# IntptrMax/YoloSharp

Measured on AMD Instinct MI355X. Metric: train images/sec YOLOv8n 640x640 bs=64/GPU, higher is better.
Workload: dtype bf16; 1 GPU; YOLOv8n detect train step (fwd+loss+bwd+AdamW), 64x3x640x640 per GPU, COCO-80 synthetic labels; global_batch=64, parallelism=dp1

## Files before the change

### yolosharp_amd/csrc/conv.hip

```cpp
#include "ys_internal.h"
#include "ys_kernels.h"
#include <atomic>
#include <cstdlib>
#include <map>
#include <mutex>
#include <vector>

template <class T, int MR, int NR, int NW>
__device__ inline void conv_epilogue(const ConvArgs& a, f32x4 (&acc)[MR][NR], const long (&orow)[MR], const bool (&mv)[MR],
                                     int n0, T* wst, float* sStat, long stat_row) {
  constexpr int EPL = Elem<T>::EPL;
  constexpr int BN = NR * 16;
  constexpr int BNP = BN + EPL;
  constexpr int VPP = BN / EPL;
  constexpr int NIT = (16 * VPP + 63) / 64;
  const int tid = threadIdx.x, lane = tid & 63, wave = tid >> 6, li = lane & 15, q = lane >> 4;
  const bool do_stats = a.stats != nullptr;
  float s1[NR][4], s2[NR][4];
#pragma unroll
  for (int nf = 0; nf < NR; nf++)
#pragma unroll
    for (int r = 0; r < 4; r++) { s1[nf][r] = 0.f; s2[nf][r] = 0.f; }
  char* yb = (char*)a.y;
  const char* rb = (const char*)a.res;
// ... 381 lines not shown
        }
#pragma unroll
        for (int nf = 0; nf < NR; nf++) {
          const uint4 wf = sW[(nf * 16 + li) * wpitch + wbase + (kh * 3 + kw) * 4 + q];
#pragma unroll
          for (int mf = 0; mf < MR; mf++) acc[mf][nf] = ys_mma<T>(wf, xf[mf], acc[mf][nf]);
        }
      }
    }
    if (chunk == nchunks - 1 && !(a.dbg & 4)) {
      __syncthreads();
      long orow[MR];
#pragma unroll
      for (int mf = 0; mf < MR; mf++) orow[mf] = (long)b * a.out_bstride + (pv[mf] ? ((long)poy[mf] * a.Wout + pox[mf]) : 0);
      T* wst = (T*)sP + wave * (16 * (BN + EPL));
      conv_epilogue<T, MR, NR, C3_THREADS / 64>(a, acc, orow, pv, n0, wst, sStat, (long)tile);
    }
    tile = ntile; chunk = nchunk;
  }
}

#include "conv_epi.h"
constexpr int YS_EPI_BATCH_P2 = 4;

#ifdef YS_P2_ABLATE
#define P2_DBG(bit) ((a.dbg & (bit)) != 0)
#else
#define P2_DBG(bit) false
#endif
constexpr int P2_KG = 2;
#define P2_NPU 12
struct P2Tag0 { static constexpr int value = 0; };
struct P2Tag1 { static constexpr int value = 1; };
__host__ __device__ constexpr int p2_reg_group(int mr, int nr, bool tight = false) {
  const int want = mr * nr >= 10 ? 1 : (mr * nr >= 6 ? 2 : 4);
  const int cap = (tight ? 8 : 16) / (mr + nr);
  const int g = want < cap ? want : cap;
  return g >= 4 ? 4 : (g >= 2 ? 2 : 1);
}
struct P2Args {
  int TH, TW, tiles_x, tiles_y, ntiles, PH, PW;
  int ppb;
  int prb;
  int wpitch;
  int nsteps;
  int nsp;
// ... 343 lines not shown
    if (WRES) ys_barrier_lds();
    TL_STAMP();

    const int rh = a.out_rh ? a.out_rh : a.Wout, rw = a.out_rh ? a.out_rw : 1;
    const int tbase = b * (int)a.out_bstride + oy0 * rh + ox0 * rw + (int)a.out_r0;
    int orow[MR];
    bool pv[MR];
#pragma unroll
    for (int mf = 0; mf < MR; mf++) {
      pv[mf] = (bool)((int)(pty[mf] < g.TH) & (int)(oy0 + pty[mf] < a.Hout) & (int)(ox0 + ptx[mf] < a.Wout));
      orow[mf] = tbase + prow[mf];
    }
    char* stg = sPb + wave * (16 * MR * (BN + 8) * 2 + 16 * MR * 16);
    if (F8) {
      const float dq = a.deq[0];
#pragma unroll
      for (int mf = 0; mf < MR; mf++)
#pragma unroll
        for (int nf = 0; nf < NR; nf++)
#pragma unroll
          for (int r = 0; r < 4; r++) acc[mf][nf][r] *= dq;
    }
#ifdef YS_P2_TIMELINE
    if (!P2_DBG(4)) p2_epilogue<MR, NR, RED, YS_EPI_BATCH_P2>(a, acc, orow, pv, n0, stg, st1, st2, [&]() { TL_STAMP(); });
#else
    if (!P2_DBG(4)) p2_epilogue<MR, NR, RED, YS_EPI_BATCH_P2>(a, acc, orow, pv, n0, stg, st1, st2);
#endif
    TL_STAMP();
    txi = ntx; tyi = nty; b = nb;
  }
  YS_WAIT_VM0();
  if (RED ? a.nred > 0 : a.stats != nullptr) p2_stats_flush<NR, NWV>(a, n0, st1, st2, (float*)sPb, (long)vbx);
  if (F8 && a.amax && blockIdx.y == 0) ys_amax_update(a.amax, amx);
  TL_STAMP();
#ifdef YS_P2_TIMELINE
  if (tl_p) tl_p[0] = (unsigned long long)tl_n;
#endif
}

template <int MR, int NR, int WRES, int NPU, int NT, int F8, int RED = 0>
__global__ void __launch_bounds__(NT, (NT == 512 ? 4 : (NPU <= 6 && MR * NR <= 8 && !F8 ? 3 : 2)))
conv_p2_kernel(ConvArgs a, P2Args g, const int* __restrict__ tab) {
  conv_p2_body<MR, NR, WRES, NPU, NT, F8, RED>(a, g, tab, (int)blockIdx.x, (int)gridDim.x);
}

struct P2Prob { ConvArgs a; P2Args g; const int* tab; };
struct P2Group { int n; int end[YS_GROUP_MAX]; P2Prob p[YS_GROUP_MAX]; };
template <int MR, int NR, int WRES, int NPU, int NT, int RED>
__global__ void __launch_bounds__(NT, (NT == 512 ? 4 : (NPU <= 6 && MR * NR <= 8 ? 3 : 2)))
// ... 299 lines not shown
  YS_LAUNCH_LDS((conv_p2_kernel<MR, NR, WRES, NPU, NT, F8, RED>), dim3(p.gx, p.gy), NT, p.lds, st, a, p.g, tab);
#ifdef YS_P2_TIMELINE
  if (tl_path) {
    static unsigned long long h[64 * 64];
    hipStreamSynchronize(st);
    hipMemcpy(h, tl_buf, sizeof(h), hipMemcpyDeviceToHost);
    FILE* f = fopen(tl_path, "a");
    if (f) {
      fprintf(f, "# k%d%d s%d cin%d cout%d M%d mr%d nr%d wres%d npu%d tile%dx%d grid%dx%d lds%d ntiles%d nsteps%d\n", a.KH, a.KW, a.SA, a.Cin, a.Cout, a.M, MR, NR, WRES, NPU, p.g.TH, p.g.TW, p.gx, p.gy, (int)p.lds, p.g.ntiles, p.g.nsteps);
      for (int w = 0; w < 64 && w * 37 < p.gx; w++) {
        const int n = (int)h[w * 64];
        if (n <= 0) continue;
        fprintf(f, "wg%d:", w * 37);
        for (int i = 1; i < n; i++) fprintf(f, " %llu", h[w * 64 + 1 + i] - h[w * 64 + 1]);
        fprintf(f, "\n");
      }
      fclose(f);
    }
  }
#endif
  return YS_OK;
}
static int conv_p2_group_dispatch(hipStream_t st, const ConvArgs* a, const P2Plan* p, int n, const int* gxs, size_t lds);
static int conv_p2_dispatch(hipStream_t st, const ConvArgs& a, const P2Plan& p) {
  {
#define P2F(M_, N_, F_, R_) { \
    if (p.wres) return p.npu == 6 ? conv_p2_launch_t<M_, N_, 1, 6, 256, F_, R_>(st, a, p) : conv_p2_launch_t<M_, N_, 1, 12, 256, F_, R_>(st, a, p); \
    return p.npu == 6 ? conv_p2_launch_t<M_, N_, 0, 6, 256, F_, R_>(st, a, p) : conv_p2_launch_t<M_, N_, 0, 12, 256, F_, R_>(st, a, p); }
#define P2(M_, N_) if (p.mr == M_ && p.nr == N_) { if (a.f8) P2F(M_, N_, 1, 0) else if (a.nred > 0) P2F(M_, N_, 0, 1) else P2F(M_, N_, 0, 0) }
    if (a.f8 && a.nred > 0) { ys_set_error("conv p2: the fused BN-backward reduction has no fp8 variant"); return YS_ERR_UNSUPPORTED; }
#ifdef YS_P2_ONE
#ifndef YS_P2_ONE_M
#define YS_P2_ONE_M 1
#define YS_P2_ONE_N 5
#endif
    P2(YS_P2_ONE_M, YS_P2_ONE_N)
#else
    P2(1, 1) P2(2, 1) P2(4, 1) P2(1, 2) P2(2, 2) P2(4, 2) P2(1, 3) P2(2, 3) P2(4, 3) P2(1, 4) P2(2, 4) P2(4, 4) P2(1, 5) P2(2, 5)
#endif
#undef P2
#undef P2F
  }
  ys_set_error("conv p2: no kernel for NT=%d MR=%d NR=%d", p.nt, p.mr, p.nr);
  return YS_ERR_UNSUPPORTED;
}


template <int MR, int NR, int WRES, int NPU, int NT, int RED>
static int conv_p2_group_launch_t(hipStream_t st, const ConvArgs* a, const P2Plan* p, int n, const int* gxs, size_t lds) {
#ifdef YS_P2_ABLATE
  const int dbg = (int)YS_OPT_INT("DBG", 0);
#else
  const int dbg = 0;
#endif
  static std::atomic<unsigned> attr_done{0};
  int dev_id = 0;
  (void)hipGetDevice(&dev_id);
  if (!(attr_done.load(std::memory_order_relaxed) & (1u << (dev_id & 31)))) {
    hipFuncSetAttribute((const void*)conv_p2_group_kernel<MR, NR, WRES, NPU, NT, RED>, hipFuncAttributeMaxDynamicSharedMemorySize, 160 * 1024);
    attr_done.fetch_or(1u << (dev_id & 31), std::memory_order_relaxed);
  }
  P2Group grp{};
  grp.n = n;
// ... 308 lines not shown
    else { if (rows_only) return 0; const int rc = conv_launch_dtype<bf16_t>(st, q); if (rc != YS_OK) return rc; }
  }
  return rows_only ? row0 - a.red_row0 : YS_OK;
}

int ys_conv_bnred_rows(const ConvArgs& a, int dtype) {
  if (dtype != YS_BF16) return 0;
  if (conv_f8_declined(a)) { ConvArgs b = a; b.f8 = 0; return ys_conv_bnred_rows(b, dtype); }
  const bool phases = ys_conv_dgrad_uses_phases(dtype, a.KH, a.DIVM + 1) && a.KW == a.KH;
  if (a.f8 && !a.x8 && a.q8 && ys_conv_wants_x8(a)) { ConvArgs b = a; b.x8 = a.q8; return ys_conv_bnred_rows(b, dtype); }
  if (phases) return conv_dgrad_s2_phases(nullptr, a, true);
  if (a.f8) {
    if (a.x8 && ys_conv_gemm_rows(a)) return a.f8 == 2 ? ys_conv_gemm_rows(a) : 0;
    const P2Plan pf = conv_p2_plan(a);
    if (pf.ok) return 0;
    ConvArgs b = a; b.f8 = 0;
    return ys_conv_bnred_rows(b, dtype);
  }
  if (ys_conv_gemm_rows(a)) return ys_conv_gemm_rows(a);
  const P2Plan p2 = conv_p2_plan(a);
  return p2.ok ? p2.gx : 0;
}

bool ys_conv_wants_x8(const ConvArgs& a) {
  if (!a.f8 || a.x8 || a.in_bstride != (long)a.Hin * a.Win) return false;
  ConvArgs b = a; b.x8 = a.x;
  if (ys_conv_dgrad_uses_phases(YS_BF16, a.KH, a.DIVM + 1) && a.KW == a.KH) {
    for (int ph = 0; ph < 4; ph++) { ConvArgs q; if (conv_dgrad_s2_phase_args(b, ph, q) && ys_conv_gemm_rows(q) != 0) return true; }
    return false;
  }
  return ys_conv_gemm_rows(b) != 0;
}

int ys_conv_launch(hipStream_t st, int dtype, const ConvArgs& a) {
  const int epl = dtype == YS_BF16 ? 8 : 4;
  if (a.Cin % epl || a.in_ldc % epl || a.in_coff % epl) {
    ys_set_error("conv: Cin/ldc/coff (%d,%d,%d) must be multiples of %d", a.Cin, a.in_ldc, a.in_coff, epl);
    return YS_ERR_INVALID_ARG;
  }
  if (dtype == YS_BF16) {
    if (conv_f8_declined(a)) { ConvArgs b = a; b.f8 = 0; return ys_conv_launch(st, dtype, b); }
    const bool phases = ys_conv_dgrad_uses_phases(dtype, a.KH, a.DIVM + 1) && a.KW == a.KH;
    if (a.f8 && !a.x8 && a.q8) {
      ConvArgs b = a; b.x8 = a.q8;
      if (ys_conv_wants_x8(a)) {
        const int rc = ys_f8_quant_view_launch(st, a.f8 == 2 ? 1 : 0, a.x, (long)a.B * a.Hin * a.Win, a.Cin, a.in_ldc, a.in_coff, a.qscale, a.q8, a.amax);
// ... 37 lines not shown
```

### yolosharp_amd/csrc/conv_epi.h

```cpp
#pragma once
#include "ys_internal.h"
#include "ys_kernels.h"

#ifdef YS_P2_ABLATE
#define EPI_DBG(bit) ((a.dbg & (bit)) != 0)
#else
#define EPI_DBG(bit) false
#endif

#include <type_traits>
template <int I, int N, class F> __device__ inline void ys_static_for(F&& f) {
  if constexpr (I < N) { f(std::integral_constant<int, I>{}); ys_static_for<I + 1, N>(f); }
}

#ifdef YS_EMU_BUILD
typedef const BnRedSeg* ys_redp_t;
__device__ inline ys_redp_t ys_red_table(const ConvArgs& a) { return a.red; }
#else
typedef const BnRedSeg __attribute__((address_space(4)))* ys_redp_t;
__device__ inline ys_redp_t ys_red_table(const ConvArgs& a) {
  const char __attribute__((address_space(4)))* ka = (const char __attribute__((address_space(4)))*)__builtin_amdgcn_kernarg_segment_ptr();
  ys_redp_t p = (ys_redp_t)(ka + a.red_koff);
  asm volatile("" : "+s"(p));
  return p;
}
#endif

__device__ inline void ys_bnred_put(const ConvArgs& a, int c, int which, long row, float t) {
  const ys_redp_t rt = ys_red_table(a);
#pragma unroll
  for (int k = 0; k < YS_BNRED_MAXSEG; k++)
    if (k < a.nred && c >= rt[k].c0 && c < rt[k].c1) {
      const int pc = c - rt[k].c0 + rt[k].yc0;
      rt[k].part[(((long)a.red_row0 + row) * 2 + which) * rt[k].C + pc] = t;
    }
}

__host__ __device__ constexpr int p2_epi_stores(int mr, int nr) { return (16 * mr + 64 / (nr * 2) - 1) / (64 / (nr * 2)); }
template <int M> struct EpiMode { static constexpr int value = M; };
struct YsNoStamp { __device__ inline void operator()() const {} };
template <int MR, int NR, int RED = 0, int BMAX = 4 , class SF = YsNoStamp>
__device__ inline void p2_epilogue(const ConvArgs& a, f32x4 (&acc)[MR][NR], const int (&orow)[MR], const bool (&pv)[MR],
                                   int n0, char* stg, float (&s1)[8], float (&s2)[8], SF stamp = SF()) {
  typedef bf16_t T;
  constexpr int BN = NR * 16;
  constexpr int PITCH = (BN + 8) * 2;
  constexpr int NPX = 16 * MR;
  constexpr int VPP = BN / 8;
  constexpr int PPI = 64 / VPP;
  constexpr int NITER = (NPX + PPI - 1) / PPI;
  static_assert(NITER == p2_epi_stores(MR, NR), "p2_epi_stores");
  const int lane = threadIdx.x & 63, li = lane & 15, q = lane >> 4;
  unsigned* rowtab = (unsigned*)(stg + NPX * PITCH);
  const int cv = lane % VPP, pl = lane / VPP;
  const bool active = lane < PPI * VPP;
  const int c = n0 + cv * 8;
  if (q == 0) {
#pragma unroll
    for (int mf = 0; mf < MR; mf++) {
      rowtab[mf * 16 + li] = pv[mf] ? ((unsigned)orow[mf] * (unsigned)a.out_ldc + (unsigned)a.out_coff) * 2u : YS_BUF_OOB;
      rowtab[NPX + mf * 16 + li] = (unsigned)orow[mf];
    }
  }
  const bool red_on = RED != 0 && a.nred > 0;
  const char* ry = nullptr; const float* rscp = nullptr; const float* rshp = nullptr; int rC = 0, rcol = 0; bool ract = false;
  uint4 yv[RED ? NITER : 1];
  float rsc[8], rsh[8];
  if (RED && red_on) {
#pragma unroll
    for (int k = 0; k < YS_BNRED_MAXSEG; k++)
      if (k < a.nred && active && c >= a.red[k].c0 && c < a.red[k].c1) {
        ry = (const char*)a.red[k].y; rscp = a.red[k].scale; rshp = a.red[k].shift; rC = a.red[k].C;
        rcol = c - a.red[k].c0 + a.red[k].yc0; ract = a.red[k].act != 0;
      }
    ys_wave_sync();
#pragma unroll
    for (int it = 0; it < NITER; it++) {
      const int px = it * PPI + pl;
      yv[it] = ys_zero16();
      if (ry && px < NPX && rowtab[px] != YS_BUF_OOB) yv[it] = ys_ld16(ry + ((long)rowtab[NPX + px] * rC + rcol) * 2L);
    }
#pragma unroll
    for (int e = 0; e < 8; e++) { rsc[e] = 0.f; rsh[e] = 0.f; }
    if (ry) { ys_ldcoef<8>(rscp + rcol, rsc); ys_ldcoef<8>(rshp + rcol, rsh); }
  }
  constexpr bool ACC_PRE = RED != 0 && NITER <= BMAX;
  uint4 ov[ACC_PRE ? NITER : 1];
  if (ACC_PRE && a.accumulate) {
    const ys_rsrcv_t rsO = ys_make_rsrcv(a.y, 0x7ffffff0u);
    if (!red_on) ys_wave_sync();
#pragma unroll
    for (int it = 0; it < NITER; it++) {
      const int px = it * PPI + pl;
      const unsigned ro = (active && px < NPX && c < a.Cout) ? rowtab[px] : YS_BUF_OOB;
      ov[it] = ys_bufld16(rsO, ro != YS_BUF_OOB ? ro + (unsigned)c * 2u : YS_BUF_OOB);
    }
  }
  stamp();
#pragma unroll
  for (int mf = 0; mf < MR; mf++) {
#pragma unroll
    for (int nf = 0; nf < NR; nf++) {
      const int c = n0 + nf * 16 + 4 * q;
      float v[4];
#pragma unroll
      for (int r = 0; r < 4; r++) v[r] = acc[mf][nf][r];
      if (!RED && !a.scale && a.shift) {
#pragma unroll
        for (int r = 0; r < 4; r++) {
          const int cc = (c + r) < a.Cout ? (c + r) : 0;
          v[r] += a.shift[cc];
        }
        if (a.act) {
#pragma unroll
          for (int r = 0; r < 4; r++) v[r] = ys_silu(v[r]);
        }
#pragma unroll
        for (int r = 0; r < 4; r++) if (c + r >= a.Cout) v[r] = 0.f;
// ... 40 lines not shown
        }
        if (bn_eval) {
#pragma unroll
          for (int e = 0; e < 8; e++) f[e] = f[e] * sc[e] + sh[e];
          if (a.act) {
#pragma unroll
            for (int e = 0; e < 8; e++) f[e] = ys_silu(f[e]);
          }
#pragma unroll
          for (int e = 0; e < 8; e++) if (c + e >= a.Cout) f[e] = 0.f;
          if (!(rb || accum)) val = ys_pack<T>(f);
        }
        T* yp = (T*)(yb + rofs + c * 2);
        if (rb || accum) {
          float gq[8];
          if (rb) {
            const long row = (long)rowtab[NPX + px];
            ys_unpack<T>(ys_ld16(rb + (row * a.res_ldc + a.res_coff + c) * 2L), gq);
#pragma unroll
            for (int e = 0; e < 8; e++) f[e] += gq[e];
          }
          if (accum) {
            if constexpr (ACC_PRE) ys_unpack<T>(ov[ACC_PRE ? it : 0], gq); else ys_unpack<T>(ys_ld16(yp), gq);
#pragma unroll
            for (int e = 0; e < 8; e++) f[e] += gq[e];
          }
          val = ys_pack<T>(f);
        }
        if (RED && red_on && ry && !EPI_DBG(512)) {
          float g[8], yf[8];
          ys_unpack<T>(val, g);
          ys_unpack<T>(yv[RED ? it : 0], yf);
          if (ract) {
#pragma unroll
            for (int e = 0; e < 8; e++) g[e] *= ys_silu_grad(yf[e] * rsc[e] + rsh[e]);
          }
#pragma unroll
          for (int e = 0; e < 8; e++) { s1[e] += g[e]; s2[e] += g[e] * yf[e]; }
        }
      }
    }
    ys_bufst16(rsY, (rofs != YS_BUF_OOB && !EPI_DBG(256)) ? rofs + (unsigned)c * 2u : YS_BUF_OOB, val);
  };
  if (EPI_DBG(1024)) { ys_wave_sync(); return; }
#pragma unroll
  for (int it = 0; it < NITER; it++) store_iter(it, EpiMode<2>{});
// ... 300 lines not shown
```

### yolosharp_amd/csrc/core.hip

```cpp
#include "ys_internal.h"
#include "ys_kernels.h"
#include <cstring>

static thread_local char g_err[1024] = "";

#include <mutex>
#include <cstdlib>
extern char** environ;
namespace {
const char* const kOptKeys[] = {"ATTN_MFMA", "BNRED", "BNRED_LOG", "BN_ATOMIC", "F8_MIN_CIN", "F8_MIN_TAPS", "GEMM_HALO", "GEMM_MIN_CIN", "GEMM_MIN_M", "GROUP", "HALO_MAX_GRID",
                                "HALO_MIN_FILL", "HALO_MR4", "HEAD_FUSE", "OVERLAP", "SPPF_FUSE", "STEM_BNB_FUSE", "STEM_DIRECT", "WGEMM_KT", "WGEMM_MIN_M", "DBG", "GEMM_DBG"};
bool opt_known(const std::string& k) {
  for (const char* n : kOptKeys) if (k == n) return true;
  return false;
}
struct OptTable {
  std::mutex mu;
  std::map<std::string, double> v;
  std::atomic<unsigned> version{1};
  OptTable() {
    for (char** e = environ; e && *e; e++) {
      if (strncmp(*e, "YS_", 3) != 0) continue;
      const char* eq = strchr(*e, '=');
      if (!eq || eq == *e + 3) continue;
      const std::string key(*e + 3, (size_t)(eq - (*e + 3)));
      if (!opt_known(key)) continue;
      char* end = nullptr;
      const double d = strtod(eq + 1, &end);
      if (end && end != eq + 1 && *end == 0) v[key] = d;
    }
  }
};
OptTable& opt_table() { static OptTable t; return t; }
}
// ... 365 lines not shown
```

### yolosharp_amd/csrc/model.hip

```cpp
#include "ys_model.h"
#include <cstring>
#include <algorithm>

namespace ysm {

static float* chan_ptr(ys_model* m, const ConvL& c, int which) { return m->chan + c.ch_off + (long)which * ((c.cout + 3) / 4 * 4); }
static char* y_ptr(const ys_model* m, const ConvL& c) { return (char*)m->y_all + (size_t)c.y_off * m->es; }
struct ResView { const void* p = nullptr; int ldc = 0, coff = 0; };
static ResView res_view(const ys_model* m, const ConvL& c) {
  if (!c.has_res) return ResView{};
  return ResView{m->bufs[c.res.buf].act, m->bufs[c.res.buf].ldc, c.res.coff};
}
static BnFinProb bn_fin(ys_model* m, const ConvL& c, const float* partial, int nblk, long count) {
  return BnFinProb{partial, nblk, c.cout, (double)count, m->params + c.g_off, m->params + c.b_off, m->state + c.rm_off, m->state + c.rv_off,
                   m->state + c.nbt_off, chan_ptr(m, c, 0), chan_ptr(m, c, 1), chan_ptr(m, c, 2), chan_ptr(m, c, 3)};
}
static int bn_finalize(ys_model* m, const ConvL& c, const float* partial, int nblk, long count) {
  const BnFinProb p = bn_fin(m, c, partial, nblk, count);
  return ys_bn_finalize_launch(m->ctx->stream, partial, nblk, c.cout, count, p.gamma, p.beta, BN_EPS, BN_MOMENTUM, p.run_mean, p.run_var, p.nbt,
                               p.scale, p.shift, p.mean, p.rstd);
}

static int run_dwconv_fwd(ys_model* m, const ConvL& c, int B) {
  hipStream_t st = m->ctx->stream;
// ... 482 lines not shown
      } else {
        rg = rb.grad; rgl = rb.ldc; rgc = c.res.coff;
      }
    }
    const bool fused = bnred_ready(c);
    if (c.pool_next) {
      const Buf& pb = m->bufs[m->pool_buf];
      const int HW = c.Hout * c.Wout;
      if ((long)B * 2 * c.cout > m->n_stat) { ys_set_error("backward: batch %d too large for the Classify statistics rows", B); return YS_ERR_STATE; }
      YS_TRY(ys_cls_bn_bwd_reduce_launch(st, m->dtype, pb.grad, pb.ldc, y, B, HW, c.cout, chan_ptr(m, c, 0), chan_ptr(m, c, 1), c.act ? 1 : 0,
                                         m->stat_partial));
      YS_TRY(bn_bwd_finalize(m, c, B, M));
      void* dyb = (m->overlap && c.dy_own) ? c.dy_own : m->dy_scratch;
      YS_TRY(ys_cls_bn_bwd_apply_launch(st, m->dtype, pb.grad, pb.ldc, y, B, HW, c.cout, chan_ptr(m, c, 0), chan_ptr(m, c, 1), chan_ptr(m, c, 4),
                                        chan_ptr(m, c, 5), c.act ? 1 : 0, dyb));
      dy = dyb; dy_ldc = c.cout; dy_coff = 0;
    } else {
    c.red_seen = 0;
    void* rg_apply = nullptr;
    if (fused) {
      const ChanFinProb p = bn_bwd_fin(m, c, bnred_src(m, c), M);
      YS_TRY(ys_bn_bwd_finalize_src_launch(st, p.src, c.cout, M, p.g0, p.g1, p.c1, p.c2, p.scale, p.mean, p.rstd));
      rg_apply = rg;
    } else {
      int nblk = 0;
      YS_TRY(ys_bn_bwd_reduce_launch(st, m->dtype, ob.grad, ob.ldc, c.out.coff, y, M, c.cout, chan_ptr(m, c, 0), chan_ptr(m, c, 1),
                                     chan_ptr(m, c, 2), chan_ptr(m, c, 3), c.act ? 1 : 0, rg, rgl, rgc, m->stat_partial, &nblk));
      YS_TRY(bn_bwd_finalize(m, c, nblk, M));
    }
    stem_fused = c.idx == 0 && m->in_f32 && c.wgp_off >= 0 && stem_bnb_planned(m);
    stem_scratch = !stem_fused && m->overlap && c.idx == 0 && !c.dy_own && !c.dw && stem_bnb_planned(m);
    void* dyb = m->dy_scratch;
    if (m->overlap && !c.dw && c.dy_own) dyb = c.dy_own;
    if (m->f8 && c.f8_bwd && m->f8_sg_valid && !c.first && !c.dw && m->q8 && m->dtype == YS_BF16 && c.cout_ld == c.cout) {
      ConvArgs q = dgrad_args(m, c, B, dyb, c.cout, 0, (long)c.Hout * c.Wout);
      f8_dgrad_operands(m, c, q);
      dy_q8 = ys_conv_wants_x8(q);
    }
    if (stem_fused) {
      if (rg_apply || dy_q8) { ys_set_error("backward: %s cannot take the fused BatchNorm backward", c.name.c_str()); return YS_ERR_STATE; }
    } else if (dy_q8) {
      YS_TRY(ys_bn_bwd_apply_q8_launch(st, ob.grad, ob.ldc, c.out.coff, y, M, c.cout, chan_ptr(m, c, 0), chan_ptr(m, c, 1), chan_ptr(m, c, 4),
                                       chan_ptr(m, c, 5), c.act ? 1 : 0, dyb, m->q8, m->f8_scales + 4L * c.idx + 2,
                                       m->amax_dy + (size_t)c.idx * YS_AMAX_WAYS, rg_apply, rgl, rgc));
    } else {
      YS_TRY(ys_bn_bwd_apply_launch(st, m->dtype, ob.grad, ob.ldc, c.out.coff, y, M, c.cout, chan_ptr(m, c, 0), chan_ptr(m, c, 1),
// ... 13 lines not shown
    if (no_dx) return YS_OK;
    int mode = 0;
    YS_TRY(claim_grad(m, c.in, &mode, c.name));
    YS_TRY(ys_dwconv_launch(st, m->dtype, 1, dy, c.cout, 0, B, c.Hin, c.Win, c.cout, m->params + c.w_off, ib.grad, ib.ldc, c.in.coff, mode));
    return YS_OK;
  }
  if (c.bn && m->overlap && dy != c.dy_own && !stem_fused && !stem_scratch) { ys_set_error("backward: %s has no dy buffer of its own", c.name.c_str()); return YS_ERR_STATE; }
  YS_TRY(queue_wgrad(m, c, B, dy, dy_ldc, dy_coff, dy_bstride, stem_fused));
  if (!c.first && !no_dx) {
    ConvArgs a = dgrad_args(m, c, B, dy, dy_ldc, dy_coff, dy_bstride);
    YS_TRY(claim_grad(m, c.in, &a.accumulate, c.name));
    if (m->f8 && c.f8_bwd) {
      unsigned* slots = m->amax_dy + (size_t)c.idx * YS_AMAX_WAYS;
      if (m->f8_sg_valid) {
        f8_dgrad_operands(m, c, a); a.amax = slots;
        a.q8 = m->q8;
        if (dy_q8) { a.x8 = m->q8; a.amax = nullptr; }
      } else {
        YS_TRY(ys_f8_view_amax_launch(st, dy, M, c.cout, dy_ldc, dy_coff, slots));
      }
    }
    if (c.bn && c.cout_ld != c.cout) { ys_set_error("backward: padded BN conv unsupported"); return YS_ERR_UNSUPPORTED; }
    attach_bnred_feeds_if_fit(m, c, a);
    YS_TRY(ys_conv_launch(st, m->dtype, a));
  }
  return YS_OK;
}

static int run_conv_bwd_group(ys_model* m, ConvL* const* cs, int n, int B) {
  hipStream_t st = m->ctx->stream;
  bool ok = n >= 2 && n <= YS_GROUP_MAX && !m->f8;
  for (int i = 0; i < n && ok; i++) {
    const ConvL& c = *cs[i];
    if (reads_detached_map(m, c)) { ok = false; break; }
    ok = !c.dw && !c.ct && !c.has_res && !c.first && c.gstat_off >= 0 && c.bn == cs[0]->bn && c.act == cs[0]->act && (!c.bn || (c.dy_own && c.cout_ld == c.cout));
    if (ok && c.bn) ok = bnred_ready(c);
  }
  if (!ok) { for (int i = 0; i < n; i++) YS_TRY(run_conv_bwd(m, *cs[i], B)); return YS_OK; }
  const void* dy[YS_GROUP_MAX]; int dy_ldc[YS_GROUP_MAX], dy_coff[YS_GROUP_MAX]; long dy_bs[YS_GROUP_MAX];
  if (cs[0]->bn) {
    ChanFinProb fp[YS_GROUP_MAX];
    BnBwdProb bp[YS_GROUP_MAX];
    for (int i = 0; i < n; i++) {
      ConvL& c = *cs[i];
      const Buf& ob = m->bufs[c.out.buf];
      const long M = (long)B * c.Hout * c.Wout;
      fp[i] = bn_bwd_fin(m, c, bnred_src(m, c), M);
      c.red_seen = 0;
// ... 175 lines not shown
```

### yolosharp_amd/csrc/plan.hip

```cpp
#include "ys_model.h"
#include <cstring>
#include <algorithm>

namespace ysm {

int dev_alloc(ys_model* m, void** p, size_t bytes, bool zero) {
  if (bytes == 0) bytes = 16;
  hipError_t e = hipMalloc(p, bytes);
  if (e != hipSuccess) { ys_set_error("hipMalloc(%zu bytes) failed: %s", bytes, hipGetErrorString(e)); return YS_ERR_OOM; }
  m->allocs.push_back(*p);
  if (zero) { e = hipMemsetAsync(*p, 0, bytes, m->ctx->stream); if (e != hipSuccess) { ys_set_error("hipMemset failed"); return YS_ERR_HIP; } }
  return YS_OK;
}

static void add_tensor(ys_model* m, const std::string& name, int kind, int conv, long off, std::vector<int64_t> shape, bool is_param) {
  TensorRec t; t.name = name; t.kind = kind; t.conv = conv; t.off = off; t.is_param = is_param;
  t.ndim = (int)shape.size(); t.count = 1;
  for (int i = 0; i < t.ndim; i++) { t.shape[i] = shape[i]; t.count *= shape[i]; }
  m->tensors.push_back(t);
}

int layout_params(ys_model* m) {
  long off = 0;
  for (int seg = 0; seg < ys_model::NSEG; seg++)
// ... 387 lines not shown
        tiles += (long)d.taps * d.tiles_ci * d.tiles_co; pt.push_back(d);
      }
    }
    if ((nf & 7) || tiles + ys_cdiv(nf / 8, 256) + ys_cdiv(pe, 256) >= (1L << 31)) ok = false;
    m->prep_fast = ok;
    if (m->prep_fast) {
      m->n_prep_tile = (int)pt.size(); m->prep_tiles = tiles; m->n_prep_phase = (int)pp.size(); m->prep_nd_phase = pe;
      if (pt.empty()) pt.push_back(PrepDesc{});
      if (pp.empty()) pp.push_back(PrepDesc{});
      YS_TRY(dev_alloc(m, (void**)&m->prep_tile_dev, pt.size() * sizeof(PrepDesc)));
      YS_TRY(dev_alloc(m, (void**)&m->prep_phase_dev, pp.size() * sizeof(PrepDesc)));
      YS_CHECK_HIP(hipMemcpyAsync(m->prep_tile_dev, pt.data(), pt.size() * sizeof(PrepDesc), hipMemcpyHostToDevice, m->ctx->stream));
      YS_CHECK_HIP(hipMemcpyAsync(m->prep_phase_dev, pp.data(), pp.size() * sizeof(PrepDesc), hipMemcpyHostToDevice, m->ctx->stream));
      YS_CHECK_HIP(hipStreamSynchronize(m->ctx->stream));
    }
  }
  YS_CHECK_HIP(hipStreamSynchronize(m->ctx->stream));
  m->n_wf_pending = nf; m->n_wd_pending = nd;
  if (m->f8) YS_TRY(alloc_f8(m, pd));
  YS_TRY(dev_alloc(m, &m->y_all, (size_t)ny * m->es));
  YS_TRY(dev_alloc(m, &m->dy_scratch, (size_t)dy_max * m->es));
  m->overlap = (YS_OPT_INT("OVERLAP", 1) != 0);
  m->overlap_built = m->overlap;
  m->stem_on = (YS_OPT_INT("STEM_DIRECT", 1) != 0);
  m->stem_bnb_fuse = (YS_OPT_INT("STEM_BNB_FUSE", 1) != 0);
  if (m->overlap) {
    {
      int least = 0, greatest = 0;
      if (hipDeviceGetStreamPriorityRange(&least, &greatest) == hipSuccess && least != greatest)
        YS_CHECK_HIP(hipStreamCreateWithPriority(&m->st2, hipStreamNonBlocking, least));
      else
        YS_CHECK_HIP(hipStreamCreateWithFlags(&m->st2, hipStreamNonBlocking));
    }
    for (auto& c : m->convs) {
      if (!c.bn || c.dw || c.ct || c.dy_own) continue;
      if (c.idx == 0 && stem_bnb_planned(m)) continue;
      YS_TRY(dev_alloc(m, &c.dy_own, (size_t)B * c.Hout * c.Wout * c.cout_ld * m->es));
    }
    for (hipEvent_t& ev : m->ev_hand) YS_CHECK_HIP(hipEventCreateWithFlags(&ev, hipEventDisableTiming));
    YS_CHECK_HIP(hipEventCreateWithFlags(&m->ev_join, hipEventDisableTiming));
  }
  for (int k = 0; k < ys_model::NSEG; k++) {
    YS_CHECK_HIP(hipEventCreateWithFlags(&m->ev_seg_m[k], hipEventDisableTiming));
    YS_CHECK_HIP(hipEventCreateWithFlags(&m->ev_seg_w[k], hipEventDisableTiming));
  }
  {
// ... 165 lines not shown
        for (auto& f : x.feeds) m->convs[f.prod].red_ok = false;
        x.feeds.clear();
        changed = true;
      }
    }
    for (auto& x : m->convs) {
      const size_t n0 = x.feeds.size();
      x.feeds.erase(std::remove_if(x.feeds.begin(), x.feeds.end(), [&](const ConvL::RedFeed& f) { return !m->convs[f.prod].red_ok; }), x.feeds.end());
      if (x.feeds.size() != n0) changed = true;
    }
  }
  long off = 0;
  for (auto& x : m->convs)
    for (size_t k = 0; k < x.feeds.size(); k++) {
      ConvL::RedFeed& f = x.feeds[k];
      f.part_off = off; off += (long)f.rows_cap * 2 * m->convs[f.prod].cout;
      m->convs[f.prod].red_src.push_back(ConvL::RedSrc{x.idx, (int)k});
    }
  for (auto& l : m->convs) {
    std::sort(l.red_src.begin(), l.red_src.end(), [&](const ConvL::RedSrc& p, const ConvL::RedSrc& q) {
      return m->convs[p.cons].feeds[p.feed].yc0 < m->convs[q.cons].feeds[q.feed].yc0; });
    if (l.red_src.empty()) l.red_ok = false;
  }
  if (off > m->n_bnred) {
    if (m->bnred_part) { YS_CHECK_HIP(hipStreamSynchronize(m->ctx->stream)); dev_free_tracked(m, m->bnred_part); m->bnred_part = nullptr; }
    YS_TRY(dev_alloc(m, (void**)&m->bnred_part, (size_t)off * 4));
    m->n_bnred = off;
  }
  if (YS_OPT_INT("BNRED_LOG", 0) != 0) {
    int nf = 0, nb = 0;
    for (auto& l : m->convs) { if (l.bn) nb++; if (l.red_ok) nf++; }
    fprintf(stderr, "[ys] fused BN-backward reduction: %d of %d BN conv units (B=%d, %.1f MB of partial rows)\n", nf, nb, B, off * 4.0 / 1e6);
    for (auto& l : m->convs) if (l.bn && !l.red_ok) fprintf(stderr, "[ys]   not fused: %s\n", l.name.c_str());
  }
  return YS_OK;
}

}
```

### yolosharp_amd/csrc/ys_kernels.h

```cpp
#pragma once
#include "ys_hip.h"

#define YS_BNRED_MAXSEG 3
#define YS_GROUP_MAX 4
#define YS_EW_GROUP_MAX 9
struct BnRedSeg {
  const void* y;
  const float* scale;
  const float* shift;
  float* part;
  int c0, c1;
  int yc0;
  int C;
  int act;
  int pad_;
};
struct ConvArgs {
  const void* x;
  const void* w;
  void* y;
  const float* scale;
  const float* shift;
  const void* res;
  float* stats;
// ... 5 lines not shown
  int out_ldc, out_coff;
  long out_bstride;
  int res_ldc, res_coff;
  int act;
  int accumulate;
  int vec_ok;
  int M;
  int TH, TW, tiles_x, tiles_y;
  int dbg;
  int pad_w_delta;
  int out_rh, out_rw;
  long out_r0;
  int f8;
  const void* w8;
  const float* qscale;
  const float* deq;
  unsigned* amax;
  void* q8;
  const void* x8;
  unsigned long long* tl;
  int nred;
  int red_row0;
  int red_koff;
  BnRedSeg red[YS_BNRED_MAXSEG];
};

struct WgradArgs {
  const void* x;
  const void* dy;
  float* partial;
  int B, Hin, Win, Cin, Hout, Wout, Cout, KH, KW, stride, pad;
  int in_ldc, in_coff;
  long in_bstride;
  int dy_ldc, dy_coff;
  long dy_bstride;
  int M;
  int dy_rh, dy_rw;
  long dy_r0;
  int TH, TWS, tiles_x, tiles_y, ntiles, PH, PW, pdb, pxb;
  unsigned dybytes, xbytes;
};

int ys_conv_launch(hipStream_t st, int dtype, const ConvArgs& a);
int ys_f8_quant_view_launch(hipStream_t st, int fmt, const void* x, long rows, int C, int ldc, int coff, const float* qscale,
                            void* out, unsigned* slots);
int ys_conv_gemm_rows(const ConvArgs& a);
bool ys_conv_wants_x8(const ConvArgs& a);
int ys_bn_act_apply_q8_launch(hipStream_t st, const void* y, long rows, int C, const float* scale, const float* shift, int act,
                              const void* res, int res_ldc, int res_coff, void* z, int z_ldc, int z_coff, void* q8,
                              const float* qscale, unsigned* amax);
int ys_bn_bwd_apply_q8_launch(hipStream_t st, const void* dz, int dz_ldc, int dz_coff, const void* y, long rows, int C,
                              const float* scale, const float* shift, const float* k2, const float* k3, int act, void* dy,
                              void* q8, const float* qscale, unsigned* amax, void* rg = nullptr, int rg_ldc = 0, int rg_coff = 0);
int ys_conv_gemm_launch(hipStream_t st, const ConvArgs& a);
bool ys_stem_eligible(int dtype, int cin, int cout, int k, int s);
int ys_stem_fwd_rows(int B, int Hout, int Wout);
int ys_stem_fwd_launch(hipStream_t st, const float* x, int B, int H, int W, const void* wf, int Cout, void* y, int out_ldc, int out_coff,
                       long out_bstride, float* stats, const float* scale, const float* shift, int act, int* rows, unsigned long long* stat_acc = nullptr);
struct StemBnb { const void* y; const float *scale, *shift, *k2, *k3; int act; };
int ys_stem_wgrad_launch(hipStream_t st, const float* x, int B, int H, int W, const void* dy, int dy_ldc, int dy_coff, long dy_bstride,
                         int Cout, float* partial, int max_splits, int* used, const StemBnb* bnb = nullptr);
int ys_conv_grid_m(const ConvArgs& a, int dtype);
int ys_conv_is_p2(const ConvArgs& a);
int ys_conv_bnred_rows(const ConvArgs& a, int dtype);
int ys_wgrad_splits(const WgradArgs& a, int dtype);
int ys_wgrad_launch(hipStream_t st, int dtype, const WgradArgs& a, int splits, int cin_real, float* grad, int* used_splits = nullptr);
#define YS_WGRED_OUT_PER_BLOCK 512
struct WgRedDesc { const float* partial; float* grad; long n; long blk0; int splits, cin_pad, cin_real, pad_; };
int ys_wgrad_reduce_batched_launch(hipStream_t st, const WgRedDesc* descs_dev, int n_desc, long total_blocks);
int ys_wgrad_gemm_splits(const WgradArgs& a);
int ys_wgrad_gemm_launch(hipStream_t st, const WgradArgs& a, int splits);
int ys_weight_prep_launch(hipStream_t st, int dtype, const float* w, int Cout, int taps, int cin_real, int cin_pad,
                          int cout_pad, void* wf, void* wd, int phase);
bool ys_conv_dgrad_uses_phases(int dtype, int k, int stride);
__host__ __device__ inline void ys_phase_wd_index(long e, int cin_real, int cout_pad, int& ci, int& tap, int& co) {
  const long blk = (long)cin_real * cout_pad;
  const int ph = e < blk ? 0 : (e < 3 * blk ? 1 : (e < 5 * blk ? 2 : 3));
  const long start = (ph == 0 ? 0 : (ph == 1 ? 1 : (ph == 2 ? 3 : 5))) * blk;
  const int pa = ph >> 1, pb = ph & 1;
  const int kwn = pb ? 2 : 1, tp_n = (pa ? 2 : 1) * kwn;
  const long el = e - start;
  co = (int)(el % cout_pad);
  const long r = el / cout_pad;
  const int tp = (int)(r % tp_n);
  ci = (int)(r / tp_n);
  const int khp = tp / kwn, kwp = tp - khp * kwn;
// ... 233 lines not shown
```

### yolosharp_amd/csrc/ys_model.h

```cpp
#pragma once
#include "ys_internal.h"
#include "ys_kernels.h"

struct View { int buf = -1; int coff = 0; int C = 0; };

struct Buf {
  int H = 0, W = 0, ldc = 0;
  long rows_per_b = 0;
  void* act = nullptr;
  void* grad = nullptr;
  bool need_grad = true;
  std::vector<char> gw;
};

struct ConvL {
  std::string name;
  int cin = 0, cout = 0, k = 1, s = 1;
  int cin_pad = 0;
  int cout_ld = 0;
  int cout_real = 0;
  bool bn = true, act = true;
  View in, out, res;
  bool has_res = false;
  int Hin = 0, Win = 0, Hout = 0, Wout = 0;
  long out_rowoff = 0;
  long w_off = -1, g_off = -1, b_off = -1;
  long rm_off = -1, rv_off = -1, nbt_off = -1;
  long wf_off = 0, wd_off = 0;
  long y_off = 0;
  long acc_off = -1;
  long ch_off = 0;
  int seg = 0;
  bool first = false;
  bool dw = false;
  bool f8_fwd = false, f8_bwd = false;
  int idx = -1, prep_idx = -1;
  long wgp_off = -1; int wgp_splits = 0;
  int red_slot = -1;
  bool proto = false;
  bool ct = false;
  struct RedFeed { int prod; int c0, c1, yc0; long part_off; int rows_cap, rows; };
  struct RedSrc { int cons, feed; };
  std::vector<RedFeed> feeds;
  std::vector<RedSrc> red_src;
  bool red_ok = false; int red_seen = 0;
  struct Member { std::string name; int row0, rows; };
  std::vector<Member> members;
  int stage = -1, group = -1;
  long gstat_off = -1;
  void* dy_own = nullptr;
  bool linear = false;
  bool pool_next = false;
};

enum OpType { OP_CONV = 0, OP_MAXPOOL = 1, OP_UPSAMPLE = 2, OP_ATTN = 3, OP_VCOPY = 4, OP_COPY = 5, OP_POOL = 6 };
struct Op { int type; int conv = -1; View in, out; int H = 0, W = 0; long aux_off = 0; int seg = 0; int heads = 0, kd = 0, hd = 0; };

struct TensorRec {
  std::string name;
  int ndim = 1; int64_t shape[4] = {1, 1, 1, 1};
  bool is_param = true;
  int kind = 0;
  int conv = -1;
  long off = 0, count = 0;
};

struct PrepDesc { long w_off, wf_off, wd_off, nf_start, nd_start; int cout, taps, cin_real, cin_pad, cout_pad, has_wd, phase;
                  long tile_start; int tiles_ci, tiles_co, layer, pad_; };
// ... 47 lines not shown
  PrepDesc* prep_tile_dev = nullptr; int n_prep_tile = 0; long prep_tiles = 0;
  PrepDesc* prep_phase_dev = nullptr; int n_prep_phase = 0; long prep_nd_phase = 0;
  bool weights_dirty = true, eval_coeffs_dirty = true;
  void* y_all = nullptr; long n_y = 0;
  void* dy_scratch = nullptr; long n_dy = 0;
  static constexpr int N_HAND = 4;
  struct PendWg { int conv; const void* dy; int ldc, coff; long bstride; bool bnb; };
  std::vector<PendWg> pend_wg; double pend_mb = 0.0; int hand_next = 0;
  bool hold_stem = false;
  hipEvent_t ev_seg_m[NSEG] = {nullptr, nullptr, nullptr, nullptr}, ev_seg_w[NSEG] = {nullptr, nullptr, nullptr, nullptr};
  bool seg_on_st2[NSEG] = {false, false, false, false};
  bool overlap = false, overlap_built = false; hipStream_t st2 = nullptr;
  hipEvent_t ev_hand[N_HAND + 1] = {nullptr}, ev_join = nullptr;
  bool st2_dirty = false;
  float* chan = nullptr; long n_chan = 0;
  float* stat_partial = nullptr; long n_stat = 0;
  unsigned long long* stat_acc_all = nullptr; long n_stat_acc = 0;
  bool bn_atomic = false;
  float* stat_group = nullptr;
  float* wg_partial = nullptr; long n_wgp = 0;
  std::vector<WgRedDesc> red_host, red_uploaded; WgRedDesc* red_dev = nullptr; int red_first[NSEG + 1] = {0, 0, 0, 0, 0}; int red_proto0 = 0;
  bool defer_wgred = true;
  bool bnred_on = true; int bnred_B = -1; float* bnred_part = nullptr; long n_bnred = 0;
  unsigned char* argmax = nullptr; long n_argmax = 0;
  float* img_dev = nullptr;
  bool stem_on = true;
  bool stem_bnb_fuse = true;
  bool sppf_fuse = true;
  const float* in_f32 = nullptr;
  float* pred = nullptr;
  float* out_stage = nullptr; long n_out_stage = 0;
  int gcap = 64; int max_labels = 0;
  float *lab_bidx = nullptr, *lab_cls = nullptr, *lab_box = nullptr;
  int* gt_count = nullptr; float* gt_box = nullptr; int* gt_cls = nullptr; float* pbox = nullptr;
  float *ov = nullptr, *align = nullptr; unsigned char* mpos = nullptr; unsigned *pos_align = nullptr, *pos_ov = nullptr;
  int* fg_gt = nullptr; float* tnorm = nullptr; float* loss_partial = nullptr; float* scalars = nullptr;
  bool e2e = false; int max_det = 300;
  void *o2o_dpd = nullptr, *o2o_dps = nullptr, *o2o_dmc = nullptr; float* scalars2 = nullptr;
  bool e2e_cv4() const { return e2e && (segment || xkind >= 2); }
  float o2m = 1.0f, o2o = 1.0f; int e2e_updates = 0, e2e_epochs = 100;
  float* det_rows = nullptr; long long* det_anchor = nullptr; void* det_ws = nullptr;
  int head_conv0 = 0, det_in[3] = {-1, -1, -1};
  long n_hstate = 0; float* hstate_snap = nullptr; unsigned char* hstate_count = nullptr;
  Range hstate_rng[4]; int n_hstate_rng = 0;
  bool e2e_pass = false;
  bool have_fwd = false, have_loss = false;
// ... 38 lines not shown
```

Measured before the change: 7391 images/s.

## Fold residual shortcut gradient into the preceding conv's dgrad epilogue

In backward, a BN conv with a residual shortcut normally hands its gradient on to the shortcut source through a separate pass (rg_apply). The shortcut share is now deferred to the dgrad of the conv that reads the same input. That dgrad's p2 epilogue loads a second accumulate operand at a byte offset (acc2_delta) and adds it while it writes out, which removes an extra read/modify/write pass over the residual gradient. Tiles with no acc2 variant fall back to an explicit copy before the conv. The change adds a new kernel template variant (RED=2), a per-plan eligibility check and an env option, and rounds the sum to bf16 before the add, so numerics shift slightly.

Result: no change. 7433 images/s (median of 6 runs) (+0.6%).

```diff
diff --git a/yolosharp_amd/csrc/conv.hip b/yolosharp_amd/csrc/conv.hip
--- a/yolosharp_amd/csrc/conv.hip
+++ b/yolosharp_amd/csrc/conv.hip
@@ -427,6 +427,9 @@
 
 #include "conv_epi.h"
 constexpr int YS_EPI_BATCH_P2 = 4;
+__host__ __device__ constexpr bool p2_acc2_variant(int mr, int nr, int wres, int npu) {
+  return nr <= 2 && mr * nr <= 4 && !(mr == 2 && nr == 2 && wres == 0 && npu == 12);
+}
 
 #ifdef YS_P2_ABLATE
 #define P2_DBG(bit) ((a.dbg & (bit)) != 0)
@@ -816,9 +819,9 @@
           for (int r = 0; r < 4; r++) acc[mf][nf][r] *= dq;
     }
 #ifdef YS_P2_TIMELINE
-    if (!P2_DBG(4)) p2_epilogue<MR, NR, RED, YS_EPI_BATCH_P2>(a, acc, orow, pv, n0, stg, st1, st2, [&]() { TL_STAMP(); });
+    if (!P2_DBG(4)) p2_epilogue<MR, NR, RED != 0 ? 1 : 0, YS_EPI_BATCH_P2, RED == 2 ? 1 : 0>(a, acc, orow, pv, n0, stg, st1, st2, [&]() { TL_STAMP(); });
 #else
-    if (!P2_DBG(4)) p2_epilogue<MR, NR, RED, YS_EPI_BATCH_P2>(a, acc, orow, pv, n0, stg, st1, st2);
+    if (!P2_DBG(4)) p2_epilogue<MR, NR, RED != 0 ? 1 : 0, YS_EPI_BATCH_P2, RED == 2 ? 1 : 0>(a, acc, orow, pv, n0, stg, st1, st2);
 #endif
     TL_STAMP();
     txi = ntx; tyi = nty; b = nb;
@@ -1164,12 +1167,23 @@
   return YS_OK;
 }
 static int conv_p2_group_dispatch(hipStream_t st, const ConvArgs* a, const P2Plan* p, int n, const int* gxs, size_t lds);
+template <int MR, int NR, int WRES, int NPU>
+static int conv_p2_launch_red(hipStream_t st, const ConvArgs& a, const P2Plan& p) {
+  if constexpr (p2_acc2_variant(MR, NR, WRES, NPU)) {
+    if (a.acc2_delta != 0) return conv_p2_launch_t<MR, NR, WRES, NPU, 256, 0, 2>(st, a, p);
+  }
+  if (a.acc2_delta != 0) { ys_set_error("conv p2: tile mr%d nr%d has no variant with a second accumulate operand", MR, NR); return YS_ERR_UNSUPPORTED; }
+  return conv_p2_launch_t<MR, NR, WRES, NPU, 256, 0, 1>(st, a, p);
+}
 static int conv_p2_dispatch(hipStream_t st, const ConvArgs& a, const P2Plan& p) {
   {
 #define P2F(M_, N_, F_, R_) { \
     if (p.wres) return p.npu == 6 ? conv_p2_launch_t<M_, N_, 1, 6, 256, F_, R_>(st, a, p) : conv_p2_launch_t<M_, N_, 1, 12, 256, F_, R_>(st, a, p); \
     return p.npu == 6 ? conv_p2_launch_t<M_, N_, 0, 6, 256, F_, R_>(st, a, p) : conv_p2_launch_t<M_, N_, 0, 12, 256, F_, R_>(st, a, p); }
-#define P2(M_, N_) if (p.mr == M_ && p.nr == N_) { if (a.f8) P2F(M_, N_, 1, 0) else if (a.nred > 0) P2F(M_, N_, 0, 1) else P2F(M_, N_, 0, 0) }
+#define P2R(M_, N_) { \
+    if (p.wres) return p.npu == 6 ? conv_p2_launch_red<M_, N_, 1, 6>(st, a, p) : conv_p2_launch_red<M_, N_, 1, 12>(st, a, p); \
+    return p.npu == 6 ? conv_p2_launch_red<M_, N_, 0, 6>(st, a, p) : conv_p2_launch_red<M_, N_, 0, 12>(st, a, p); }
+#define P2(M_, N_) if (p.mr == M_ && p.nr == N_) { if (a.f8) P2F(M_, N_, 1, 0) else if (a.nred > 0) P2R(M_, N_) else P2F(M_, N_, 0, 0) }
     if (a.f8 && a.nred > 0) { ys_set_error("conv p2: the fused BN-backward reduction has no fp8 variant"); return YS_ERR_UNSUPPORTED; }
 #ifdef YS_P2_ONE
 #ifndef YS_P2_ONE_M
@@ -1181,6 +1195,7 @@
     P2(1, 1) P2(2, 1) P2(4, 1) P2(1, 2) P2(2, 2) P2(4, 2) P2(1, 3) P2(2, 3) P2(4, 3) P2(1, 4) P2(2, 4) P2(4, 4) P2(1, 5) P2(2, 5)
 #endif
 #undef P2
+#undef P2R
 #undef P2F
   }
   ys_set_error("conv p2: no kernel for NT=%d MR=%d NR=%d", p.nt, p.mr, p.nr);
@@ -1535,6 +1550,14 @@
   return p2.ok ? p2.gx : 0;
 }
 
+bool ys_conv_takes_acc2(const ConvArgs& a, int dtype) {
+  if (dtype != YS_BF16 || a.f8 || !a.accumulate || a.nred <= 0) return false;
+  if (ys_conv_dgrad_uses_phases(dtype, a.KH, a.DIVM + 1) && a.KW == a.KH) return false;
+  if (ys_conv_gemm_rows(a)) return false;
+  const P2Plan p2 = conv_p2_plan(a);
+  return p2.ok && p2.nt == 256 && p2_epi_stores(p2.mr, p2.nr) <= YS_EPI_BATCH_P2 && p2_acc2_variant(p2.mr, p2.nr, p2.wres ? 1 : 0, p2.npu);
+}
+
 bool ys_conv_wants_x8(const ConvArgs& a) {
   if (!a.f8 || a.x8 || a.in_bstride != (long)a.Hin * a.Win) return false;
   ConvArgs b = a; b.x8 = a.x;
diff --git a/yolosharp_amd/csrc/conv_epi.h b/yolosharp_amd/csrc/conv_epi.h
--- a/yolosharp_amd/csrc/conv_epi.h
+++ b/yolosharp_amd/csrc/conv_epi.h
@@ -9,6 +9,7 @@
 #endif
 
 #include <type_traits>
+#include <cstddef>
 template <int I, int N, class F> __device__ inline void ys_static_for(F&& f) {
   if constexpr (I < N) { f(std::integral_constant<int, I>{}); ys_static_for<I + 1, N>(f); }
 }
@@ -26,6 +27,15 @@
 }
 #endif
 
+static_assert(offsetof(ConvArgs, red) == offsetof(ConvArgs, acc2_delta) + sizeof(int), "acc2_delta sits directly in front of the segment table");
+__device__ inline int ys_acc2_delta(const ConvArgs& a) {
+#ifdef YS_EMU_BUILD
+  return a.acc2_delta;
+#else
+  return *(const int __attribute__((address_space(4)))*)((const char __attribute__((address_space(4)))*)ys_red_table(a) - sizeof(int));
+#endif
+}
+
 __device__ inline void ys_bnred_put(const ConvArgs& a, int c, int which, long row, float t) {
   const ys_redp_t rt = ys_red_table(a);
 #pragma unroll
@@ -39,7 +49,8 @@
 __host__ __device__ constexpr int p2_epi_stores(int mr, int nr) { return (16 * mr + 64 / (nr * 2) - 1) / (64 / (nr * 2)); }
 template <int M> struct EpiMode { static constexpr int value = M; };
 struct YsNoStamp { __device__ inline void operator()() const {} };
-template <int MR, int NR, int RED = 0, int BMAX = 4 , class SF = YsNoStamp>
+template <int MR, int NR, int RED = 0, int BMAX = 4 ,
+          int A2 = 0 , class SF = YsNoStamp>
 __device__ inline void p2_epilogue(const ConvArgs& a, f32x4 (&acc)[MR][NR], const int (&orow)[MR], const bool (&pv)[MR],
                                    int n0, char* stg, float (&s1)[8], float (&s2)[8], SF stamp = SF()) {
   typedef bf16_t T;
@@ -85,15 +96,20 @@
     if (ry) { ys_ldcoef<8>(rscp + rcol, rsc); ys_ldcoef<8>(rshp + rcol, rsh); }
   }
   constexpr bool ACC_PRE = RED != 0 && NITER <= BMAX;
+  constexpr bool ACC2 = ACC_PRE && A2 != 0;
   uint4 ov[ACC_PRE ? NITER : 1];
+  uint4 ov2[ACC2 ? NITER : 1];
+  int d2 = 0;
   if (ACC_PRE && a.accumulate) {
     const ys_rsrcv_t rsO = ys_make_rsrcv(a.y, 0x7ffffff0u);
     if (!red_on) ys_wave_sync();
+    if constexpr (ACC2) d2 = ys_acc2_delta(a);
 #pragma unroll
     for (int it = 0; it < NITER; it++) {
       const int px = it * PPI + pl;
       const unsigned ro = (active && px < NPX && c < a.Cout) ? rowtab[px] : YS_BUF_OOB;
       ov[it] = ys_bufld16(rsO, ro != YS_BUF_OOB ? ro + (unsigned)c * 2u : YS_BUF_OOB);
+      if constexpr (ACC2) ov2[it] = ys_bufld16(rsO, (ro != YS_BUF_OOB && d2 != 0) ? ro + (unsigned)c * 2u + (unsigned)d2 : YS_BUF_OOB);
     }
   }
   stamp();
@@ -180,6 +196,15 @@
           }
           if (accum) {
             if constexpr (ACC_PRE) ys_unpack<T>(ov[ACC_PRE ? it : 0], gq); else ys_unpack<T>(ys_ld16(yp), gq);
+            if constexpr (ACC2) {
+              if (d2 != 0) {
+                float g2[8];
+                ys_unpack<T>(ov2[ACC2 ? it : 0], g2);
+#pragma unroll
+                for (int e = 0; e < 8; e++) gq[e] += g2[e];
+                ys_unpack<T>(ys_pack<T>(gq), gq);
+              }
+            }
 #pragma unroll
             for (int e = 0; e < 8; e++) f[e] += gq[e];
           }
diff --git a/yolosharp_amd/csrc/core.hip b/yolosharp_amd/csrc/core.hip
--- a/yolosharp_amd/csrc/core.hip
+++ b/yolosharp_amd/csrc/core.hip
@@ -9,7 +9,7 @@
 extern char** environ;
 namespace {
 const char* const kOptKeys[] = {"ATTN_MFMA", "BNRED", "BNRED_LOG", "BN_ATOMIC", "F8_MIN_CIN", "F8_MIN_TAPS", "GEMM_HALO", "GEMM_MIN_CIN", "GEMM_MIN_M", "GROUP", "HALO_MAX_GRID",
-                                "HALO_MIN_FILL", "HALO_MR4", "HEAD_FUSE", "OVERLAP", "SPPF_FUSE", "STEM_BNB_FUSE", "STEM_DIRECT", "WGEMM_KT", "WGEMM_MIN_M", "DBG", "GEMM_DBG"};
+                                "HALO_MIN_FILL", "HALO_MR4", "HEAD_FUSE", "OVERLAP", "RES_DGRAD", "SPPF_FUSE", "STEM_BNB_FUSE", "STEM_DIRECT", "WGEMM_KT", "WGEMM_MIN_M", "DBG", "GEMM_DBG"};
 bool opt_known(const std::string& k) {
   for (const char* n : kOptKeys) if (k == n) return true;
   return false;
diff --git a/yolosharp_amd/csrc/model.hip b/yolosharp_amd/csrc/model.hip
--- a/yolosharp_amd/csrc/model.hip
+++ b/yolosharp_amd/csrc/model.hip
@@ -528,6 +528,7 @@
       const ChanFinProb p = bn_bwd_fin(m, c, bnred_src(m, c), M);
       YS_TRY(ys_bn_bwd_finalize_src_launch(st, p.src, c.cout, M, p.g0, p.g1, p.c1, p.c2, p.scale, p.mean, p.rstd));
       rg_apply = rg;
+      if (rg && c.res_to >= 0 && !m->f8) { m->convs[c.res_to].res_due = (c.out.coff - c.res.coff) * (int)m->es; rg_apply = nullptr; }
     } else {
       int nblk = 0;
       YS_TRY(ys_bn_bwd_reduce_launch(st, m->dtype, ob.grad, ob.ldc, c.out.coff, y, M, c.cout, chan_ptr(m, c, 0), chan_ptr(m, c, 1),
@@ -587,8 +588,17 @@
     }
     if (c.bn && c.cout_ld != c.cout) { ys_set_error("backward: padded BN conv unsupported"); return YS_ERR_UNSUPPORTED; }
     attach_bnred_feeds_if_fit(m, c, a);
+    if (c.res_due) {
+      if (ys_conv_takes_acc2(a, m->dtype)) a.acc2_delta = c.res_due;
+      else {
+        const ConvL& l = m->convs[c.res_from];
+        YS_TRY(ys_copy_view_launch(st, m->dtype, m->bufs[l.out.buf].grad, m->bufs[l.out.buf].ldc, l.out.coff, M, l.cout, ib.grad, ib.ldc, c.in.coff, 1));
+      }
+      c.res_due = 0;
+    }
     YS_TRY(ys_conv_launch(st, m->dtype, a));
   }
+  if (c.res_due) { ys_set_error("backward: %s did not take the shortcut share it was left", c.name.c_str()); return YS_ERR_STATE; }
   return YS_OK;
 }
 
diff --git a/yolosharp_amd/csrc/plan.hip b/yolosharp_amd/csrc/plan.hip
--- a/yolosharp_amd/csrc/plan.hip
+++ b/yolosharp_amd/csrc/plan.hip
@@ -433,6 +433,7 @@
   YS_TRY(dev_alloc(m, &m->dy_scratch, (size_t)dy_max * m->es));
   m->overlap = (YS_OPT_INT("OVERLAP", 1) != 0);
   m->overlap_built = m->overlap;
+  m->res_dgrad = (YS_OPT_INT("RES_DGRAD", 1) != 0);
   m->stem_on = (YS_OPT_INT("STEM_DIRECT", 1) != 0);
   m->stem_bnb_fuse = (YS_OPT_INT("STEM_BNB_FUSE", 1) != 0);
   if (m->overlap) {
@@ -644,6 +645,21 @@
       return m->convs[p.cons].feeds[p.feed].yc0 < m->convs[q.cons].feeds[q.feed].yc0; });
     if (l.red_src.empty()) l.red_ok = false;
   }
+  for (auto& c : m->convs) { c.res_to = -1; c.res_from = -1; c.res_due = 0; }
+  if (m->res_dgrad && !m->f8) {
+    for (size_t oi = 1; oi < m->ops.size(); oi++) {
+      if (m->ops[oi].type != OP_CONV || m->ops[oi - 1].type != OP_CONV) continue;
+      ConvL& l = m->convs[m->ops[oi].conv];
+      ConvL& x = m->convs[m->ops[oi - 1].conv];
+      if (!l.bn || !l.has_res || l.dw || l.ct || l.pool_next || l.group >= 0 || l.res.buf != l.out.buf || l.res.C != l.out.C || l.cout_ld != l.cout) continue;
+      if (x.dw || x.ct || x.first || x.s != 1 || x.group >= 0 || x.feeds.empty()) continue;
+      if (x.in.buf != l.res.buf || x.in.coff != l.res.coff || x.in.C != l.res.C || x.cin_pad != l.res.C || x.Hin != l.Hout || x.Win != l.Wout) continue;
+      if ((long)B * m->bufs[l.out.buf].rows_per_b * m->bufs[l.out.buf].ldc * 2 >= (1L << 31) - 16) continue;
+      ConvArgs a = dgrad_plan_args(m, x, B, false);
+      a.accumulate = 1; a.nred = (int)x.feeds.size();
+      if (ys_conv_takes_acc2(a, m->dtype)) { l.res_to = x.idx; x.res_from = l.idx; }
+    }
+  }
   if (off > m->n_bnred) {
     if (m->bnred_part) { YS_CHECK_HIP(hipStreamSynchronize(m->ctx->stream)); dev_free_tracked(m, m->bnred_part); m->bnred_part = nullptr; }
     YS_TRY(dev_alloc(m, (void**)&m->bnred_part, (size_t)off * 4));
@@ -654,6 +670,9 @@
     for (auto& l : m->convs) { if (l.bn) nb++; if (l.red_ok) nf++; }
     fprintf(stderr, "[ys] fused BN-backward reduction: %d of %d BN conv units (B=%d, %.1f MB of partial rows)\n", nf, nb, B, off * 4.0 / 1e6);
     for (auto& l : m->convs) if (l.bn && !l.red_ok) fprintf(stderr, "[ys]   not fused: %s\n", l.name.c_str());
+    int ns = 0, nd = 0;
+    for (auto& l : m->convs) { if (l.bn && l.has_res) ns++; if (l.res_to >= 0) nd++; }
+    fprintf(stderr, "[ys] shortcut share on the dgrad: %d of %d shortcut units\n", nd, ns);
   }
   return YS_OK;
 }
diff --git a/yolosharp_amd/csrc/ys_kernels.h b/yolosharp_amd/csrc/ys_kernels.h
--- a/yolosharp_amd/csrc/ys_kernels.h
+++ b/yolosharp_amd/csrc/ys_kernels.h
@@ -51,6 +51,7 @@
   int nred;
   int red_row0;
   int red_koff;
+  int acc2_delta;
   BnRedSeg red[YS_BNRED_MAXSEG];
 };
 
@@ -91,6 +92,7 @@
                          int Cout, float* partial, int max_splits, int* used, const StemBnb* bnb = nullptr);
 int ys_conv_grid_m(const ConvArgs& a, int dtype);
 int ys_conv_is_p2(const ConvArgs& a);
+bool ys_conv_takes_acc2(const ConvArgs& a, int dtype);
 int ys_conv_bnred_rows(const ConvArgs& a, int dtype);
 int ys_wgrad_splits(const WgradArgs& a, int dtype);
 int ys_wgrad_launch(hipStream_t st, int dtype, const WgradArgs& a, int splits, int cin_real, float* grad, int* used_splits = nullptr);
diff --git a/yolosharp_amd/csrc/ys_model.h b/yolosharp_amd/csrc/ys_model.h
--- a/yolosharp_amd/csrc/ys_model.h
+++ b/yolosharp_amd/csrc/ys_model.h
@@ -44,6 +44,7 @@
   std::vector<RedFeed> feeds;
   std::vector<RedSrc> red_src;
   bool red_ok = false; int red_seen = 0;
+  int res_to = -1, res_from = -1, res_due = 0;
   struct Member { std::string name; int row0, rows; };
   std::vector<Member> members;
   int stage = -1, group = -1;
@@ -137,6 +138,7 @@
   std::vector<WgRedDesc> red_host, red_uploaded; WgRedDesc* red_dev = nullptr; int red_first[NSEG + 1] = {0, 0, 0, 0, 0}; int red_proto0 = 0;
   bool defer_wgred = true;
   bool bnred_on = true; int bnred_B = -1; float* bnred_part = nullptr; long n_bnred = 0;
+  bool res_dgrad = true;
   unsigned char* argmax = nullptr; long n_argmax = 0;
   float* img_dev = nullptr;
   bool stem_on = true;
```
